# luisdiaz1997/GPzoo

Hardware: AMD Instinct MI355X
Metric: ELBO evals/sec (L=32-latent evaluations, all GPUs) at M=2048 inducing, N=200000, L=32 latents/GPU x 1 GPU(s) (higher is better)
Workload: dtype f32; 1 GPU; BASELINE configs[2]: Slide-seq-shaped synthetic, N=200000 spots, M=2048, L=32 latents/GPU x 1 GPU(s), matern32, f32; latents_total=32, whitened=True, chunk=0, factor_dtype=f64

## Files before the change

### gpzoo_amd/build.py

```python
from __future__ import annotations

import os
import subprocess
import sys

HERE = os.path.dirname(os.path.abspath(__file__))
CSRC = os.path.join(HERE, "csrc")
LIB = os.path.join(HERE, "libgpzoo_hip.so")
SOURCES = ["runtime.hip", "kfill.hip", "gemm.hip", "gemmw.hip", "gemmp.hip", "diag128.hip", "coop.hip", "factor.hip", "kgrad.hip", "mmops.hip", "poisson.hip", "svgp.hip", "vnngp.hip", "collective.hip", "spatial.hip", "nmf.hip", "smooth.hip", "kmeans.hip", "gram.hip", "poisson_sparse.hip", "nmf_sparse.hip", "deviance.hip", "nb.hip", "nb_sparse.hip", "nb_deviance.hip", "gaussian.hip", "gaussian_sparse.hip", "gene_rank.hip", "gene_dispersion.hip", "residual.hip", "moran_perm.hip", "spatial_stats.hip"]
HEADERS = ["common.h", "vec.h", "sparse_rows.h", "gene_rows.h", "moran_expr.h", "nb_passes.h", "moran_pass.h", "residual_gaussian.h", "gemm.h", "cov.h", "gemmw.h", "gemmp.h", "diag128.h", "factor.h", "kgrad.h", "mmops.h", os.path.join("..", "..", "include", "gpzoo_hip.h")]
FLAGS = ["--offload-arch=gfx950", "-O3", "-std=c++17", "-fPIC", "-ffp-contract=fast", "-Wall", "-Wno-unused-function"]
SOURCE_FLAGS = {"spatial.hip": ["-ffp-contract=off"], "smooth.hip": ["-ffp-contract=off"], "kmeans.hip": ["-ffp-contract=off"],
                "gene_rank.hip": ["-ffp-contract=off"], "gene_dispersion.hip": ["-ffp-contract=off"],
                "residual.hip": ["-ffp-contract=off"], "moran_perm.hip": ["-ffp-contract=off"],
                "spatial_stats.hip": ["-ffp-contract=off"]}


HASH_MARK = b"GPZ_SRC_HASH:"


def source_hash():
    import hashlib
    h = hashlib.sha256()
    for f in sorted(SOURCES + HEADERS):
        path = os.path.join(CSRC, f)
        if not os.path.exists(path):
            return None
        h.update(os.path.basename(f).encode() + b"\0")
        h.update(open(path, "rb").read())
        h.update(b"\0")
    return h.hexdigest()[:32]


def embedded_hash(lib_path: str = LIB):
    try:
        blob = open(lib_path, "rb").read()
    except OSError:
        return None
    i = blob.find(HASH_MARK)
    if i < 0:
        return None
    j = blob.find(b"\0", i)
    return blob[i + len(HASH_MARK):j].decode("ascii", "replace")
# ... 40 lines not shown
```

### gpzoo_amd/csrc/gemmw.h

```cpp
#pragma once
#include "common.h"

namespace gpz {

struct Fused1Args {
  const float* Linv; int64_t Mp;
  const float* Z; int64_t M;
  const float* X; int64_t nreal;
  int d, kind, L;
  const float* sigma; const float* ell;
  float* Wt; int64_t ncp;
  const float* muE;
  float* ps_sq; float* ps_mu;
};
bool fused1_supported(int dtype, int kind, int d);
int fused1_launch(const Fused1Args& a, hipStream_t s);

enum WideEpilogue {
  WIDE_STORE_STATS = 0,
  WIDE_STATS = 1,
  WIDE_STORE = 2,
  WIDE_STORE_COLSCALE = 3,
  WIDE_WBAR = 4,
  WIDE_KBAR = 5,
  WIDE_ADD_COLSCALE = 6,
};
struct WideArgs {
  const float* A; const float* B; int64_t Mp, ncp; int L;
  int upper, epilogue;
  float* C; const float* mu;
  float* ps_sq; float* ps_mu;
  const float* colscale; const float* colvec;
  const float* rowvec;
  const float* aux;
  const int32_t* gate;
};
bool wide_product_supported(int64_t Mp, int64_t ncp);
int wide_product_launch(const WideArgs& a, hipStream_t s);

bool wide_nt_supported(int64_t Mp, int64_t K);
int wide_nt_pieces(int64_t Mp, int64_t K, int L);
size_t wide_nt_scratch_floats(int64_t Mp, int64_t K, int L);
size_t wide_nt_vpart_floats(int64_t Mp, int64_t K, int L);
int wide_nt_launch(const float* A, const float* B, float* C, int64_t Mp, int64_t K, int L, hipStream_t s, float* scratch = nullptr,
                   const float* w = nullptr, const int32_t* gate = nullptr, const float* gm = nullptr, float* vpart = nullptr,
                   double* v = nullptr, int64_t v_stride = 0);

}
```

### gpzoo_amd/csrc/gemmw.hip

```cpp
#include "gemmw.h"

#include "cov.h"


#include <cmath>
#include <mutex>
#include <type_traits>
#include <utility>

#ifndef GPZ_W_ABL
#define GPZ_W_ABL 0
#endif

namespace gpz {

typedef float f32x4 __attribute__((ext_vector_type(4)));

enum { WB_MEM = 0, WB_GEN = 1 };
enum { WA_DENSE = 0, WA_LOWER = 1, WA_UPPER = 2 };
enum { WE_STORE_STATS = 0,
       WE_STATS = 1,
       WE_STORE = 2,
       WE_STORE_COLSCALE = 3,
       WE_WBAR = 4,
       WE_KBAR = 5,
       WE_ADD_COLSCALE = 6 };

struct WParams {
  const float* A; int64_t lda, sA0;
  const float* B; int64_t ldb, sB0;
  const float* Z; int64_t MD;
  const float* X; int64_t nreal;
  const float* sigma; const float* ell;
  float* C; int64_t ldc, sC0;
  const float* mu; int64_t sMu;
  float* ps_sq; float* ps_mu; int64_t ncols;
  const float* colscale; const float* colvec; int64_t sCs;
  const float* rowvec; int64_t sRv;
  const float* aux;
  int64_t M;
  int L, nblk, mtw, nt, W, strips;
  int pair, colmajor;
  const int32_t* gate;
};

constexpr int W_BK = 16;

template <int TM, int TN, int BSRC, int D>
struct WLds {
  static constexpr int A_ELEMS = TM * W_BK;
  static constexpr int RPP = 256 / TN;
  static constexpr int PITCH = 256 + (RPP == 2 ? 8 : RPP == 1 ? 4 : 16);
  static constexpr int B_ELEMS = (W_BK / RPP) * PITCH;
  static constexpr int STAGE = A_ELEMS + B_ELEMS;
  static constexpr int ZB = 128 * D;
  static constexpr size_t bytes = sizeof(float) * (2 * STAGE + (BSRC == WB_GEN ? 2 * ZB : 0));
};

template <int TM, int TN, int BSRC, int ATRI, int EPI, int KIND, int D>
// ... 222 lines not shown
    active = db < p.nblk && (int64_t)tj * TN + wn * 32 < p.ncols;
    n_a = 8 * (ATRI == WA_LOWER ? db : wm);
    fr_a = (wm * 128 + r) * BK + ((q ^ gperm(r)) * 4);
    step0 = k_begin / BK;
    t = 0;
    next_ti = leg + 1 < nlegs ? leg_ti[leg + 1] : -1;
#pragma unroll
    for (int mi = 0; mi < 8; ++mi)
#pragma unroll
      for (int ni = 0; ni < 2; ++ni) acc[mi][ni] = f32x4{0, 0, 0, 0};
    if constexpr (BSRC == WB_GEN) {
      z_load(step0 >> 3);
      asm volatile("s_waitcnt vmcnt(0)" ::: "memory");
      __syncthreads();
      b_generate(0, step0);
    }
    if (leg == 0) asm volatile("s_waitcnt vmcnt(0)" ::: "memory");
    asm volatile("s_waitcnt lgkmcnt(0)" ::: "memory");
    __builtin_amdgcn_s_barrier();
    if (!active) {
      idle_until(nk);
    } else if constexpr (ATRI == WA_DENSE) {
      full_until(nk);
    } else if constexpr (ATRI == WA_LOWER) {
      full_until(n_a);
      diagonal(diagonal, i0{});
      idle_until(nk);
    } else {
      idle_until(n_a);
      diagonal(diagonal, i0{});
      full_until(nk);
    }

    if (!active) continue;
    if (GPZ_W_ABL & 4) {
      float sum = 0.f;
#pragma unroll
      for (int mi = 0; mi < 8; ++mi)
#pragma unroll
        for (int ni = 0; ni < 2; ++ni)
#pragma unroll
          for (int g = 0; g < 4; ++g) sum += acc[mi][ni][g];
      if (sum == 12345.678f) p.ps_sq[0] = sum;
      continue;
    }
    const int64_t row0 = (int64_t)db * 128;
    const int64_t ccol0 = (int64_t)tj * TN + wn * 32;
    if (BSRC == WB_GEN && row0 + 128 > p.M) {
#pragma unroll
      for (int mi = 0; mi < 8; ++mi)
#pragma unroll
        for (int g = 0; g < 4; ++g)
          if (row0 + mi * 16 + 4 * q + g >= p.M) {
#pragma unroll
            for (int ni = 0; ni < 2; ++ni) acc[mi][ni][g] = 0.f;
          }
    }
    if constexpr (EPI == WE_STORE_STATS || EPI == WE_STATS) {
      float ssq[2] = {0.f, 0.f}, smu[2] = {0.f, 0.f};
#pragma unroll
      for (int mi = 0; mi < 8; ++mi) {
        f32x4 m4 = {0, 0, 0, 0};
        if constexpr (EPI == WE_STORE_STATS) m4 = *reinterpret_cast<const f32x4*>(p.mu + b0 * p.sMu + row0 + 4 * q + mi * 16);
#pragma unroll
        for (int g = 0; g < 4; ++g)
#pragma unroll
          for (int ni = 0; ni < 2; ++ni) {
            const float v = acc[mi][ni][g];
            ssq[ni] = __builtin_fmaf(v, v, ssq[ni]);
            if constexpr (EPI == WE_STORE_STATS) smu[ni] = __builtin_fmaf(m4[g], v, smu[ni]);
          }
      }
#pragma unroll
      for (int ni = 0; ni < 2; ++ni) {
        ssq[ni] += __shfl_xor(ssq[ni], 16); ssq[ni] += __shfl_xor(ssq[ni], 32);
        if constexpr (EPI == WE_STORE_STATS) { smu[ni] += __shfl_xor(smu[ni], 16); smu[ni] += __shfl_xor(smu[ni], 32); }
        if (q == 0) {
          const int64_t o = ((int64_t)b0 * p.nblk + db) * p.ncols + ccol0 + ni * 16 + r;
          p.ps_sq[o] = ssq[ni];
          if constexpr (EPI == WE_STORE_STATS) p.ps_mu[o] = smu[ni];
        }
      }
    }
    if constexpr (EPI != WE_STATS) {
      constexpr int LDE = 36;
      static_assert(NW * 16 * LDE <= G::STAGE, "the epilogue strips fit tile buffer 1");
      float* strip = sA(1) + wave * (16 * LDE);
      float* Cg = p.C + b0 * p.sC0 + row0 * p.ldc + ccol0;
      int srow = lane >> 3;
      asm volatile("" : "+v"(srow));
      const int c4 = (lane & 7) * 4;
      float cs[2] = {1.f, 1.f};
      if constexpr (EPI == WE_STORE_COLSCALE) {
#pragma unroll
        for (int ni = 0; ni < 2; ++ni) cs[ni] = p.colscale[b0 * p.sCs + ccol0 + ni * 16 + r];
      }
      f32x4 sc = {0, 0, 0, 0}, cv = {0, 0, 0, 0};
      if constexpr (EPI == WE_WBAR || EPI == WE_KBAR || EPI == WE_ADD_COLSCALE)
        sc = *reinterpret_cast<const f32x4*>(p.colscale + b0 * p.sCs + ccol0 + c4);
      if constexpr (EPI == WE_WBAR || EPI == WE_KBAR)
        cv = *reinterpret_cast<const f32x4*>(p.colvec + b0 * p.sCs + ccol0 + c4);
#pragma unroll
      for (int mi = 0; mi < 8; ++mi) {
#pragma unroll
        for (int ni = 0; ni < 2; ++ni)
#pragma unroll
          for (int g = 0; g < 4; ++g) strip[(4 * q + g) * LDE + ni * 16 + r] = cs[ni] * acc[mi][ni][g];
        __builtin_amdgcn_wave_barrier();
        f32x4 w[2];
        float rv[2];
        if constexpr (EPI == WE_WBAR || EPI == WE_KBAR || EPI == WE_ADD_COLSCALE) {
#pragma unroll
          for (int it = 0; it < 2; ++it) {
            const int64_t row = mi * 16 + it * 8 + srow;
            if constexpr (EPI == WE_WBAR) w[it] = *reinterpret_cast<const f32x4*>(p.aux + b0 * p.sC0 + (row0 + row) * p.ldc + ccol0 + c4);
            if constexpr (EPI == WE_ADD_COLSCALE) w[it] = *reinterpret_cast<const f32x4*>(Cg + (int64_t)row * p.ldc + c4);
            if constexpr (EPI != WE_ADD_COLSCALE) rv[it] = p.rowvec[b0 * p.sRv + row0 + row];
// ... 325 lines not shown
  GPZ_REQUIRE(fused1_supported(GPZ_F32, a.kind, a.d), "fused stage 1: kind=%d d=%d unsupported", a.kind, a.d);
  GPZ_REQUIRE(a.Mp % 128 == 0 && a.ncp % 128 == 0 && a.Mp > 0 && a.ncp > 0 && a.L > 0, "fused stage 1: bad extents");
  GPZ_REQUIRE(a.Mp * a.Mp * 4 < (1ll << 31) && a.M * a.d * 4 < (1ll << 31), "fused stage 1: M too large");
  constexpr int TM = 512, TN = 128;
  WParams p = {};
  p.A = a.Linv; p.lda = a.Mp; p.sA0 = a.Mp * a.Mp;
  p.Z = a.Z; p.MD = a.M * a.d; p.M = a.M;
  p.X = a.X; p.nreal = a.nreal;
  p.sigma = a.sigma; p.ell = a.ell;
  p.C = a.Wt; p.ldc = a.ncp; p.sC0 = a.Mp * a.ncp;
  p.mu = a.muE; p.sMu = a.Mp;
  p.ps_sq = a.ps_sq; p.ps_mu = a.ps_mu; p.ncols = a.ncp;
  p.L = a.L; p.nblk = (int)(a.Mp / 128); p.mtw = (int)((a.Mp + TM - 1) / TM); p.nt = (int)(a.ncp / TN);
  int strips = (p.nt + 31) / 32;
  const int want = (32 + p.mtw * p.L - 1) / (p.mtw * p.L);
  if (strips < want) strips = want < p.nt ? want : p.nt;
  p.W = (p.nt + strips - 1) / strips;
  p.strips = (p.nt + p.W - 1) / p.W;
  const int64_t units = (int64_t)p.mtw * p.L * p.strips;
  const int64_t nblocks = (units + 7) / 8 * 8 * p.W;
#define GPZ_W1(KIND, D) return launch_wide(gemmw_kernel<TM, TN, WB_GEN, WA_LOWER, WE_STORE_STATS, KIND, D>, \
                                           WLds<TM, TN, WB_GEN, D>::bytes, p, nblocks, s, 1024)
  if (a.kind == GPZ_KERNEL_MATERN32) { if (a.d == 2) GPZ_W1(1, 2); GPZ_W1(1, 1); }
  if (a.kind == GPZ_KERNEL_MATERN12) { if (a.d == 2) GPZ_W1(4, 2); GPZ_W1(4, 1); }
  if (a.kind == GPZ_KERNEL_MATERN52) { if (a.d == 2) GPZ_W1(5, 2); GPZ_W1(5, 1); }
  if (a.d == 2) GPZ_W1(0, 2);
  GPZ_W1(0, 1);
#undef GPZ_W1
}

bool wide_product_supported(int64_t Mp, int64_t ncp) {
  return Mp % 128 == 0 && ncp % 128 == 0 && Mp * Mp * 4 < (1ll << 31) && Mp * ncp * 4 < (1ll << 31);
}

template <int TM, int TN>
static int wide_product_launch_t(const WideArgs& a, hipStream_t s) {
  WParams p = {};
  p.A = a.A; p.lda = a.Mp; p.sA0 = a.Mp * a.Mp;
  p.B = a.B; p.ldb = a.ncp; p.sB0 = a.Mp * a.ncp;
  p.C = a.C; p.ldc = a.ncp; p.sC0 = a.Mp * a.ncp;
  p.mu = a.mu; p.sMu = a.Mp;
  p.ps_sq = a.ps_sq; p.ps_mu = a.ps_mu; p.ncols = a.ncp; p.M = a.Mp;
  p.colscale = a.colscale; p.colvec = a.colvec; p.sCs = a.ncp; p.rowvec = a.rowvec; p.sRv = a.Mp; p.aux = a.aux;
  p.gate = a.gate;
  p.L = a.L; p.nblk = (int)(a.Mp / 128); p.mtw = (int)((a.Mp + TM - 1) / TM); p.nt = (int)((a.ncp + TN - 1) / TN);
  constexpr int WMAX = 4096 / TN;
  int strips = (p.nt + WMAX - 1) / WMAX;
  const int want = (8 + p.L - 1) / p.L;
  if (strips < want) strips = want < p.nt ? want : p.nt;
  p.strips = strips;
  p.W = (p.nt + strips - 1) / strips;
  const int64_t units = (int64_t)p.L * p.strips;
  const int64_t paired = (units + 7) / 8 * 8 * ((p.mtw + 1) / 2) * p.W;
  p.pair = p.colmajor = paired >= 4 * 512;
  const int64_t nblocks = p.pair ? paired : (units + 7) / 8 * 8 * p.mtw * p.W;
  constexpr size_t lds = WLds<TM, TN, WB_MEM, 1>::bytes;
#define GPZ_WM(ATRI, EPI) return launch_wide(gemmw_kernel<TM, TN, WB_MEM, ATRI, EPI, 0, 1>, lds, p, nblocks, s)
  switch (a.epilogue) {
    case WIDE_STORE_STATS:
      GPZ_REQUIRE(!a.upper && a.C && a.mu && a.ps_sq && a.ps_mu, "wide product: store + statistics is the lower-triangular product and needs C, mu and both slabs");
      GPZ_WM(WA_LOWER, WE_STORE_STATS);
    case WIDE_STATS:
      GPZ_REQUIRE(a.upper && a.ps_sq, "wide product: statistics only is the upper-triangular product");
      GPZ_WM(WA_UPPER, WE_STATS);
    case WIDE_STORE:
      GPZ_REQUIRE(a.upper && a.C, "wide product: the plain store is built for the upper-triangular product");
      GPZ_WM(WA_UPPER, WE_STORE);
    case WIDE_STORE_COLSCALE:
      GPZ_REQUIRE(a.upper && a.C && a.colscale, "wide product: the column-scaled store is the upper-triangular product and needs the factors");
      GPZ_WM(WA_UPPER, WE_STORE_COLSCALE);
    case WIDE_WBAR:
      GPZ_REQUIRE(!a.upper && a.C && a.colscale && a.colvec && a.rowvec && a.aux, "wide product: the W-bar epilogue needs its operands");
      GPZ_WM(WA_LOWER, WE_WBAR);
    case WIDE_KBAR:
      GPZ_REQUIRE(a.upper == 2 && a.C && a.colscale && a.colvec && a.rowvec, "wide product: the K-bar epilogue is the dense product and needs its vectors");
      GPZ_WM(WA_DENSE, WE_KBAR);
    case WIDE_ADD_COLSCALE:
      GPZ_REQUIRE(a.upper == 1 && a.C && a.colscale, "wide product: the accumulating column-scaled store is the upper-triangular product");
      GPZ_WM(WA_UPPER, WE_ADD_COLSCALE);
    default: break;
  }
#undef GPZ_WM
  GPZ_REQUIRE(false, "wide product: unknown epilogue %d", a.epilogue);
}

int wide_product_launch(const WideArgs& a, hipStream_t s) {
  GPZ_REQUIRE(wide_product_supported(a.Mp, a.ncp) && a.L > 0, "wide product: bad extents");
  return wide_product_launch_t<128, 256>(a, s);
}

bool wide_nt_supported(int64_t Mp, int64_t K) {
  return Mp % 128 == 0 && K % 128 == 0 && K > 0 && Mp * K * 4 < (1ll << 31);
}

static bool nt_small_tiles(int64_t nblk) { return nblk <= 4; }
static int64_t nt_tiles(int64_t nblk) {
  if (nt_small_tiles(nblk)) return nblk * (nblk + 1) / 2;
  const int64_t mt = (nblk + 1) / 2;
  return mt * (mt + 1) - (nblk & 1);
}

int wide_nt_pieces(int64_t Mp, int64_t K, int L) {
  const int64_t tiles = nt_tiles(Mp / 128) * L;
  if (tiles >= 384) {
    const double r = (double)tiles / 512.0;
    int best = 1;
    double best_cost = 1e30;
    for (int S = 1; S <= 4; ++S) {
      if (S > 1 && K / S < 2048) break;
      const double rounds = r * S, cost = std::ceil(rounds - 1e-9) / rounds * (1.0 + 0.015 * (S - 1));
      if (cost < best_cost - 1e-9) { best_cost = cost; best = S; }
    }
// ... 56 lines not shown
```

### gpzoo_amd/csrc/kgrad.h

```cpp
#pragma once
#include "common.h"

namespace gpz {

struct KgradArgs {
  const void* Kbar; int64_t ld, stride;
  const void* Z; const void* X;
  const int64_t* gZ; const int64_t* gX;
  const void* sigma; const void* ell; const void* ga; const void* gr2;
  double gpow, scalar_scale;
  int64_t M, ncols, Mp;
  int d, G;
  double* acc;
};

int kgrad_launch(int dtype, int kind, const KgradArgs& a, int L, hipStream_t s);

}
```

### gpzoo_amd/csrc/kgrad.hip

```cpp
#include "kgrad.h"
#include "mmops.h"

namespace gpz {

__device__ __forceinline__ float kg_exp(float x) { return __builtin_amdgcn_exp2f(x * 1.44269504088896341f); }
__device__ __forceinline__ double kg_exp(double x) { return exp(x); }
__device__ __forceinline__ float kg_sqrt(float x) { return sqrtf(x); }
__device__ __forceinline__ double kg_sqrt(double x) { return sqrt(x); }
__device__ __forceinline__ float kg_rsqrt(float x) { return rsqrtf(x); }
__device__ __forceinline__ double kg_rsqrt(double x) { return 1.0 / sqrt(x); }
__device__ __forceinline__ float kg_pow(float x, float y) { return __builtin_amdgcn_exp2f(y * __builtin_amdgcn_logf(x)); }
__device__ __forceinline__ double kg_pow(double x, double y) { return pow(x, y); }

template <typename T, int KIND>
__global__ __launch_bounds__(256) void kgrad_kernel(KgradArgs a) {
  const int l = blockIdx.y, wave = threadIdx.x >> 6, lane = threadIdx.x & 63;
  const int64_t m = (int64_t)blockIdx.x * 4 + wave;
  if (m >= a.M) return;
  const T* kb = static_cast<const T*>(a.Kbar) + (int64_t)l * a.stride + m * a.ld;
  const T* Zp = static_cast<const T*>(a.Z);
  const T* Xp = static_cast<const T*>(a.X);
  const int d = a.d;
  const T sig = static_cast<const T*>(a.sigma)[l];
  const T ell = static_cast<const T*>(a.ell)[l];
  const T s2 = sig * sig, il2 = (T)1 / (ell * ell);
  T z[4] = {0, 0, 0, 0};
  for (int k = 0; k < d; ++k) z[k] = Zp[m * d + k];
  const int gz = (KIND == 2) ? ((uint64_t)a.gZ[m] < (uint64_t)a.G ? (int)a.gZ[m] : 0) : 0;
  const T aeff = (KIND == 2) ? static_cast<const T*>(a.ga)[l] : (T)0;
  const T gpow = (T)a.gpow;
  double dz[4] = {0, 0, 0, 0}, dsig = 0, dell = 0, da = 0;
  constexpr int UN = 4;
  for (int64_t c0 = lane; c0 < a.ncols; c0 += 64 * UN) {
    T g[UN], x[UN][4];
    int gx[UN];
#pragma unroll
    for (int u = 0; u < UN; ++u) {
      const int64_t c = c0 + 64 * u;
      const bool in = c < a.ncols;
      g[u] = in ? kb[c] : (T)0;
#pragma unroll
      for (int k = 0; k < 4; ++k) x[u][k] = (in && k < d) ? Xp[c * d + k] : (T)0;
      gx[u] = (KIND == 2 && in) ? ((uint64_t)a.gX[c] < (uint64_t)a.G ? (int)a.gX[c] : 0) : 0;
    }
    T pz[4] = {0, 0, 0, 0}, psig = 0, pell = 0, pa = 0;
#pragma unroll
    for (int u = 0; u < UN; ++u) {
      T diff[4], d2 = 0;
#pragma unroll
      for (int k = 0; k < 4; ++k) { diff[k] = (k < d) ? z[k] - x[u][k] : (T)0; d2 = fma(diff[k], diff[k], d2); }
      T cz;
      if (KIND == 0) {
        const T kv = s2 * kg_exp((T)-0.5 * d2 * il2);
        psig += g[u] * (T)2 * kv / sig;
        pell += g[u] * kv * d2 * il2 / ell;
        cz = -kv * il2;
      } else if (KIND == 1) {
        const T v = (T)1.7320508075688772935 * kg_sqrt(d2) / ell, e = kg_exp(-v);
        psig += g[u] * (T)2 * sig * ((T)1 + v) * e;
        pell += g[u] * s2 * v * v * e / ell;
        cz = -s2 * (T)3 * il2 * e;
      } else if (KIND == 4) {
        const T rr = kg_sqrt(d2), kv = s2 * kg_exp(-rr / ell);
        psig += g[u] * (T)2 * kv / sig;
        pell += g[u] * kv * rr * il2;
        cz = d2 > (T)0 ? -(kv / ell) * kg_rsqrt(d2) : (T)0;
      } else if (KIND == 5) {
        const T v = (T)2.2360679774997896964 * kg_sqrt(d2) / ell, e = kg_exp(-v), q3 = v * v / (T)3;
        psig += g[u] * (T)2 * sig * ((T)1 + v + q3) * e;
        pell += g[u] * s2 * q3 * ((T)1 + v) * e / ell;
        cz = -s2 * (T)5 / (T)3 * il2 * ((T)1 + v) * e;
      } else {
        const T r2 = static_cast<const T*>(a.gr2)[gz * a.G + gx[u]];
        const T den = aeff * r2 + (T)1;
        const T kv = s2 * kg_exp((T)-0.5 * d2 * il2 / den) * kg_pow(den, -gpow);
        psig += g[u] * (T)2 * kv / sig;
        pell += g[u] * kv * d2 * il2 / (ell * den);
        pa += g[u] * kv * ((T)0.5 * d2 * il2 / (den * den) - gpow / den) * r2;
        cz = -kv * il2 / den;
      }
      const T gc = g[u] * cz;
#pragma unroll
      for (int k = 0; k < 4; ++k) pz[k] = fma(gc, diff[k], pz[k]);
    }
    dsig += (double)psig; dell += (double)pell; da += (double)pa;
#pragma unroll
    for (int k = 0; k < 4; ++k) dz[k] += (double)pz[k];
  }
  double v[7] = {dz[0], dz[1], dz[2], dz[3], dsig * a.scalar_scale, dell * a.scalar_scale, da * a.scalar_scale};
#pragma unroll
  for (int i = 0; i < 7; ++i)
    for (int o = 32; o > 0; o >>= 1) v[i] += __shfl_down(v[i], o);
  if (lane == 0) {
    double* dst = a.acc + ((int64_t)l * a.Mp + m) * 8;
#pragma unroll
    for (int i = 0; i < 7; ++i) dst[i] += v[i];
  }
}

int kgrad_launch(int dtype, int kind, const KgradArgs& a, int L, hipStream_t s) {
  GPZ_REQUIRE((kind >= 0 && kind <= 2) || kind == GPZ_KERNEL_MATERN12 || kind == GPZ_KERNEL_MATERN52,
              "kgrad: unknown kernel kind %d", kind);
  dim3 grid((unsigned)((a.M + 3) / 4), (unsigned)L), block(256);
#define GPZ_KG(T, K) hipLaunchKernelGGL((kgrad_kernel<T, K>), grid, block, 0, s, a)
#define GPZ_KG_KINDS(T) \
  switch (kind) { case 0: GPZ_KG(T, 0); break; case 1: GPZ_KG(T, 1); break; case 4: GPZ_KG(T, 4); break; \
                  case 5: GPZ_KG(T, 5); break; default: GPZ_KG(T, 2); break; }
  if (dtype == GPZ_F32) GPZ_KG_KINDS(float) else GPZ_KG_KINDS(double)
#undef GPZ_KG_KINDS
#undef GPZ_KG
  GPZ_LAUNCH_OK();
  return 0;
}

}

extern "C" size_t gpz_kgrad_workspace_bytes(int64_t nA, int32_t n_latent) {
  if (nA < 1 || n_latent < 1) return 0;
  gpz::Carver c(nullptr);
  c.take<double>((int64_t)n_latent * nA * 8);
  return c.used();
}

extern "C" int gpz_kgrad(const gpz_kernel_desc* k, const void* A, int64_t nA, const void* B, int64_t nB, int32_t d,
                         const int64_t* gA, const int64_t* gB, const void* Kbar, int64_t ldk, int64_t stride_k,
                         double* grad_theta, double* grad_A, void* ws, size_t ws_bytes, void* stream) {
  using namespace gpz;
  GPZ_REQUIRE(k && A && B && Kbar && ws, "gpz_kgrad: null pointer");
  GPZ_REQUIRE(nA >= 1 && nB >= 1 && ldk >= nB && d >= 1 && d <= 4, "gpz_kgrad: bad extents nA=%lld nB=%lld ldk=%lld d=%d",
              (long long)nA, (long long)nB, (long long)ldk, d);
  GPZ_REQUIRE((k->kind >= 0 && k->kind <= 2) || k->kind == GPZ_KERNEL_MATERN12 || k->kind == GPZ_KERNEL_MATERN52,
              "gpz_kgrad: kernel kind %d has no parameters to differentiate", k->kind);
  GPZ_REQUIRE(k->n_latent >= 1 && (k->dtype == GPZ_F32 || k->dtype == GPZ_F64), "gpz_kgrad: bad kernel description");
  if (k->kind == GPZ_KERNEL_MGGP_RBF)
    GPZ_REQUIRE(gA && gB && k->group_a && k->group_r2 && k->n_groups >= 1, "gpz_kgrad: MGGP kernel needs groups, group_a, group_r2");
  GPZ_REQUIRE(ws_bytes >= gpz_kgrad_workspace_bytes(nA, k->n_latent), "gpz_kgrad: workspace too small");
  hipStream_t s = static_cast<hipStream_t>(stream);
  const int L = k->n_latent;
  Carver c(ws);
  double* acc = c.take<double>((int64_t)L * nA * 8);
  GPZ_HIP_OK(hipMemsetAsync(acc, 0, sizeof(double) * L * nA * 8, s));
  KgradArgs a;
  a.Kbar = Kbar; a.ld = ldk; a.stride = stride_k; a.Z = A; a.X = B; a.gZ = gA; a.gX = gB;
  a.sigma = k->sigma; a.ell = k->lengthscale; a.ga = k->group_a; a.gr2 = k->group_r2;
  a.gpow = k->group_pow; a.scalar_scale = 1.0; a.M = nA; a.ncols = nB; a.Mp = nA; a.d = d; a.G = k->n_groups; a.acc = acc;
  if (int rc = kgrad_launch(k->dtype, k->kind, a, L, s)) return rc;
  return kgrad_finish(acc, L, nA, nA, d, nullptr, grad_A, grad_theta, s);
// ... 2 lines not shown
```

### gpzoo_amd/csrc/svgp.hip

```cpp
#include "common.h"
#include "gemmw.h"
#include "gemmp.h"
#include "factor.h"
#include "gemm.h"
#include "kgrad.h"
#include "mmops.h"

#include <algorithm>
#include <cstdlib>
#include <cstring>

namespace gpz {

constexpr int NB = 128;

struct ProductSchedule { int cols, tpw; };
template <typename T>
static ProductSchedule product_schedule(bool stats_epilogue, int nt) {
  const int tpw = (sizeof(T) == 4 && stats_epilogue) ? 2 : 1;
  const int full = 16 * tpw;
  const int strips = (nt + full - 1) / full;
  int w = (nt + strips * tpw - 1) / (strips * tpw);
  if (w > 16) w = 16;
  return ProductSchedule{w * tpw, tpw};
// ... 845 lines not shown
    b.any_d = c.take<int32_t>(pl.nchunks + 1);
  }
  b.bytes = c.used();
  return b;
}

template <typename TR, typename T>
__global__ __launch_bounds__(256) void q_finish_kernel(TR* __restrict__ R, const T* __restrict__ Hd, int64_t Mp, int64_t M,
                                                      const double* __restrict__ u, const double* __restrict__ v) {
  const int l = blockIdx.z;
  const int64_t i = blockIdx.y, j = (int64_t)blockIdx.x * 256 + threadIdx.x;
  if (j >= Mp || (j >> 7) > (i >> 7)) return;
  const int64_t o = (int64_t)l * Mp * Mp + i * Mp + j;
  double r = (double)R[o];
  if (Hd) r += (double)Hd[o];
  if (i < M && j < M) r += u[(int64_t)l * Mp + i] * v[(int64_t)l * Mp + j];
  R[o] = (TR)r;
}
template <typename T>
__global__ void minus_identity_t_kernel(T* __restrict__ A, int64_t Mp) {
  const int l = blockIdx.y;
  const int64_t i = (int64_t)blockIdx.x * 256 + threadIdx.x;
  if (i < Mp) A[(int64_t)l * Mp * Mp + i * (Mp + 1)] -= (T)1;
}

static bool backward_algebra(int64_t N, int64_t Mp, bool full, int flags, bool f64_algebra) {
  static const int env = [] { const char* e = getenv("GPZ_SVGP_BACKWARD"); return !e ? 0 : !strcmp(e, "algebra") ? 1 : !strcmp(e, "classic") ? 2 : 0; }();
  if (flags & GPZ_SVGP_BACKWARD_ALGEBRA) return true;
  if (flags & GPZ_SVGP_BACKWARD_CLASSIC) return false;
  if (env) return env == 1;
  return full ? 10 * N >= (f64_algebra ? 44 : 22) * Mp : 4 * N >= 3 * Mp;
}

template <typename T>
static int svgp_backward_t(const gpz_svgp_problem* p, const gpz_svgp_grads* g, int64_t chunk, void* ws, size_t ws_bytes,
                           hipStream_t s) {
  const Plan pl = make_plan(p, chunk);
  const bool wh = p->whitened != 0;
  const bool full = g->grad_theta != nullptr || g->grad_Z != nullptr;
  Buffers<T> b = carve<T>(pl, wh, ws);
  BwdBuffers<T> w = carve_bwd<T>(pl, wh, full, ws, b.bytes);
  GPZ_REQUIRE(ws_bytes >= w.bytes, "gpz_svgp_backward: workspace too small (%zu < %zu)", ws_bytes, w.bytes);
  const int64_t L = pl.L, M = pl.M, Mp = pl.Mp, N = pl.N, mm = Mp * Mp;
  const int L32 = (int)L;
  const bool alg64 = sizeof(T) == 4 && !wh;
  const bool alg = backward_algebra(N, Mp, full, p->flags, alg64);
  gpz_svgp_problem q = *p;
  q.chol = nullptr; q.Lu = nullptr;
  if (int rc = prepare_t<T>(&q, pl, b, s)) return rc;
  {
    Zeroer z;
    if (alg) z.add(w.H, sizeof(T) * L * mm);
    z.add(w.G, sizeof(T) * L * mm);
    if (!wh) z.add(w.G2, sizeof(T) * L * mm);
    if (full) {
      if (alg && wh) {
        z.add(w.Hd, sizeof(T) * L * mm);
        z.add(w.any_d, sizeof(int32_t) * (pl.nchunks + 1));
      }
      if (!alg) z.add(w.GL, sizeof(T) * L * mm);
      z.add(w.kacc, sizeof(double) * L * Mp * 8);
      z.add(w.sig_direct, sizeof(double) * L);
    }
    if (int rc = z.run(s)) return rc;
  }
  const dim3 g32((unsigned)(Mp / 32), (unsigned)(Mp / 32), L32);
// ... 124 lines not shown
      if (with_hd)
        if (int rc = syrk(w.csd, w.Hd, w.any_d + ci)) return rc;
      v_done = wide_nt;
    } else {
      bool done = false;
      if constexpr (sizeof(T) == 4) {
        if (wide) {
          WideArgs wa = {};
          wa.A = b.LuT; wa.B = Wc; wa.Mp = Mp; wa.ncp = ncp; wa.L = L32; wa.upper = 1; wa.epilogue = WIDE_STORE_COLSCALE;
          wa.C = w.Pc; wa.colscale = w.cs;
          if (int rc = wide_product_launch(wa, s)) return rc;
          done = true;
        }
      }
      if (!done) {
        GemmParams<T> g2;
        g2.A = b.LuT; g2.lda = Mp; g2.sA0 = mm;
        g2.B = Wc; g2.ldb = ncp; g2.sB0 = Mp * ncp;
        g2.C = w.Pc; g2.ldc = ncp; g2.sC0 = Mp * ncp;
        g2.nb0 = L32; g2.mt = (int)pl.nblk; g2.nt = nt; g2.K = (int)Mp; g2.flags = GF_A_UPPER | GF_GROUP_COLS;
        g2.super_cols = sched_plain.cols; g2.colscale = w.cs; g2.sCs = ncp; g2.ncols = ncp;
        if (int rc = gemm_launch(g2, EPI_STORE_COLSCALE, s)) return rc;
      }
      if (wide_nt) {
        if constexpr (sizeof(T) == 4) { if (int rc = wide_nt_launch(Wc, w.Pc, w.G, Mp, ncp, L32, s, w.nt_part)) return rc; }
      } else if (int rc = nt_generic(Wc, w.Pc, w.G)) return rc;
    }
    if (!v_done) {
      hipLaunchKernelGGL((rowdot_kernel<T>), dim3((unsigned)(Mp / 4), L32), dim3(256), 0, s, Wc, Mp, ncp,
                         static_cast<const T*>(g->g_mean), N, n0, w.mu_part, pl.nchunks, ci);
      GPZ_LAUNCH_OK();
    }
    if (full) {
      bool done = false;
      if constexpr (sizeof(T) == 4) {
        if (wide && alg) {
          WideArgs wk = {};
          wk.A = w.A1; wk.B = Wc; wk.Mp = Mp; wk.ncp = ncp; wk.L = L32; wk.upper = 2; wk.epilogue = WIDE_KBAR;
          wk.C = w.Pc; wk.colscale = w.cs; wk.colvec = w.gmc; wk.rowvec = w.a3;
          if (int rc = wide_product_launch(wk, s)) return rc;
          if (with_hd) {
            WideArgs wc = {};
            wc.A = w.LinvT; wc.B = Wc; wc.Mp = Mp; wc.ncp = ncp; wc.L = L32; wc.upper = 1; wc.epilogue = WIDE_ADD_COLSCALE;
            wc.C = w.Pc; wc.colscale = w.csd; wc.gate = w.any_d + ci;
            if (int rc = wide_product_launch(wc, s)) return rc;
          }
          done = true;
        }
        if (wide && !alg) {
          WideArgs wa = {};
          wa.A = w.LuN; wa.B = w.Pc; wa.Mp = Mp; wa.ncp = ncp; wa.L = L32; wa.upper = 0; wa.epilogue = WIDE_WBAR;
          wa.C = b.Kc; wa.colscale = w.csc; wa.colvec = w.gmc; wa.rowvec = b.muE; wa.aux = Wc;
          if (int rc = wide_product_launch(wa, s)) return rc;
          WideArgs wb = {};
          wb.A = w.LinvT; wb.B = b.Kc; wb.Mp = Mp; wb.ncp = ncp; wb.L = L32; wb.upper = 1; wb.epilogue = WIDE_STORE;
          wb.C = w.Pc;
          if (int rc = wide_product_launch(wb, s)) return rc;
          done = true;
        }
      }
      if (!done) {
        if (alg) {
          GemmParams<T> g2;
          g2.A = b.LuT; g2.lda = Mp; g2.sA0 = mm;
          g2.B = Wc; g2.ldb = ncp; g2.sB0 = Mp * ncp;
          g2.C = w.Pc; g2.ldc = ncp; g2.sC0 = Mp * ncp;
          g2.nb0 = L32; g2.mt = (int)pl.nblk; g2.nt = nt; g2.K = (int)Mp; g2.flags = GF_A_UPPER | GF_GROUP_COLS;
          g2.super_cols = sched_plain.cols; g2.colscale = w.cs; g2.sCs = ncp; g2.ncols = ncp;
          if (int rc = gemm_launch(g2, EPI_STORE_COLSCALE, s)) return rc;
        }
        GemmParams<T> g4;
        g4.A = w.LuN; g4.lda = Mp; g4.sA0 = mm;
        g4.B = w.Pc; g4.ldb = ncp; g4.sB0 = Mp * ncp;
        g4.C = b.Kc; g4.ldc = ncp; g4.sC0 = Mp * ncp;
        g4.nb0 = L32; g4.mt = (int)pl.nblk; g4.nt = nt; g4.K = (int)Mp; g4.flags = GF_A_LOWER | GF_GROUP_COLS;
        g4.super_cols = sched_plain.cols; g4.colscale = w.csc; g4.colvec = w.gmc; g4.sCs = ncp; g4.rowvec = b.muE; g4.sRv = Mp;
        g4.aux = Wc; g4.ncols = ncp;
        if (int rc = gemm_launch(g4, EPI_WBAR, s)) return rc;
        GemmParams<T> g5;
        g5.A = w.LinvT; g5.lda = Mp; g5.sA0 = mm;
        g5.B = b.Kc; g5.ldb = ncp; g5.sB0 = Mp * ncp;
        g5.C = w.Pc; g5.ldc = ncp; g5.sC0 = Mp * ncp;
        g5.nb0 = L32; g5.mt = (int)pl.nblk; g5.nt = nt; g5.K = (int)Mp; g5.flags = GF_A_UPPER | GF_GROUP_COLS;
        g5.super_cols = sched_plain.cols;
        if (int rc = gemm_launch(g5, EPI_STORE, s)) return rc;
      }
      if (!alg) {
        if (wide_nt) {
          if constexpr (sizeof(T) == 4) { if (int rc = wide_nt_launch(w.Pc, Wc, w.GL, Mp, ncp, L32, s, w.nt_part)) return rc; }
        } else if (int rc = nt_generic(w.Pc, Wc, w.GL)) return rc;
      }
      KgradArgs ka;
      ka.Kbar = w.Pc; ka.ld = ncp; ka.stride = Mp * ncp; ka.Z = p->Z; ka.X = Xc;
      ka.gZ = p->gZ; ka.gX = p->gX ? p->gX + n0 : nullptr;
      ka.sigma = p->k.sigma; ka.ell = p->k.lengthscale; ka.ga = p->k.group_a; ka.gr2 = p->k.group_r2;
      ka.gpow = p->k.group_pow; ka.scalar_scale = 1.0; ka.M = M; ka.ncols = nreal; ka.Mp = Mp; ka.d = p->d;
      ka.G = p->k.n_groups; ka.acc = w.kacc;
      if (int rc = kgrad_launch(p->dtype, p->k.kind, ka, L32, s)) return rc;
      hipLaunchKernelGGL((sigma_direct_kernel<T>), dim3(L32), dim3(256), 0, s, w.csc, ncp,
                         static_cast<const T*>(p->k.sigma), w.sig_direct);
      GPZ_LAUNCH_OK();
    }
  }
  hipLaunchKernelGGL(chunk_sum_kernel, dim3((unsigned)((Mp + 255) / 256), L32), dim3(256), 0, s, w.mu_part, pl.nchunks,
                     Mp, w.mu_sum);
  GPZ_LAUNCH_OK();
  if (alg) {
    hipLaunchKernelGGL((mirror_lower_kernel<T>), g32, dim3(256), 0, s, w.H, Mp);
    GPZ_LAUNCH_OK();
    if (int rc = tgemm(w.H, b.LuT, w.G, GF_B_TRANS | GF_B_LOWER | GF_TILES_LOWER)) return rc;
    if (full) {
      if (alg64) {
        hipLaunchKernelGGL((widen_kernel<T>), dim3(2048), dim3(256), 0, s, (const T*)w.H, w.D1, L * mm, 0);
        GPZ_LAUNCH_OK();
        if (int rc = dgemm(w.D2, w.D1, w.D3, GF_TILES_LOWER)) return rc;
        hipLaunchKernelGGL((q_finish_kernel<double, T>), gm, dim3(256), 0, s, w.D3, (const T*)nullptr, Mp, M,
                           (const double*)w.me, (const double*)w.mu_sum);
        GPZ_LAUNCH_OK();
        if (int rc = tril_transpose(b.Linv, Mp, L32, w.D1, s)) return rc;
        if (int rc = dgemm(w.D1, w.D3, w.D4, GF_A_UPPER | GF_TILES_LOWER)) return rc;
      } else {
        if (int rc = tgemm(w.SwI, w.H, w.PS, GF_TILES_LOWER)) return rc;
        hipLaunchKernelGGL((q_finish_kernel<T, T>), gm, dim3(256), 0, s, w.PS, wh ? (const T*)w.Hd : (const T*)nullptr, Mp, M,
                           (const double*)w.me, (const double*)w.mu_sum);
        GPZ_LAUNCH_OK();
        if (int rc = tgemm(w.LinvT, w.PS, w.GL, GF_A_UPPER | GF_TILES_LOWER)) return rc;
      }
    }
  }
  const double* g_kl = g->g_kl;
  if (g_kl && !wh) {
// ... 263 lines not shown
```

Baseline: 2.650 ELBO evals/s.

## Fuse kernel-gradient contraction into wide K-bar product epilogue

Result: no change. 2.645 ELBO evals/s (-0.2%).

```diff
diff --git a/gpzoo_amd/build.py b/gpzoo_amd/build.py
--- a/gpzoo_amd/build.py
+++ b/gpzoo_amd/build.py
@@ -8,7 +8,7 @@
 CSRC = os.path.join(HERE, "csrc")
 LIB = os.path.join(HERE, "libgpzoo_hip.so")
 SOURCES = ["runtime.hip", "kfill.hip", "gemm.hip", "gemmw.hip", "gemmp.hip", "diag128.hip", "coop.hip", "factor.hip", "kgrad.hip", "mmops.hip", "poisson.hip", "svgp.hip", "vnngp.hip", "collective.hip", "spatial.hip", "nmf.hip", "smooth.hip", "kmeans.hip", "gram.hip", "poisson_sparse.hip", "nmf_sparse.hip", "deviance.hip", "nb.hip", "nb_sparse.hip", "nb_deviance.hip", "gaussian.hip", "gaussian_sparse.hip", "gene_rank.hip", "gene_dispersion.hip", "residual.hip", "moran_perm.hip", "spatial_stats.hip"]
-HEADERS = ["common.h", "vec.h", "sparse_rows.h", "gene_rows.h", "moran_expr.h", "nb_passes.h", "moran_pass.h", "residual_gaussian.h", "gemm.h", "cov.h", "gemmw.h", "gemmp.h", "diag128.h", "factor.h", "kgrad.h", "mmops.h", os.path.join("..", "..", "include", "gpzoo_hip.h")]
+HEADERS = ["common.h", "vec.h", "sparse_rows.h", "gene_rows.h", "moran_expr.h", "nb_passes.h", "moran_pass.h", "residual_gaussian.h", "gemm.h", "cov.h", "gemmw.h", "gemmp.h", "diag128.h", "factor.h", "kgrad.h", "kgrad_terms.h", "mmops.h", os.path.join("..", "..", "include", "gpzoo_hip.h")]
 FLAGS = ["--offload-arch=gfx950", "-O3", "-std=c++17", "-fPIC", "-ffp-contract=fast", "-Wall", "-Wno-unused-function"]
 SOURCE_FLAGS = {"spatial.hip": ["-ffp-contract=off"], "smooth.hip": ["-ffp-contract=off"], "kmeans.hip": ["-ffp-contract=off"],
                 "gene_rank.hip": ["-ffp-contract=off"], "gene_dispersion.hip": ["-ffp-contract=off"],
diff --git a/gpzoo_amd/csrc/gemmw.h b/gpzoo_amd/csrc/gemmw.h
--- a/gpzoo_amd/csrc/gemmw.h
+++ b/gpzoo_amd/csrc/gemmw.h
@@ -24,6 +24,8 @@
   WIDE_WBAR = 4,
   WIDE_KBAR = 5,
   WIDE_ADD_COLSCALE = 6,
+  WIDE_KBAR_CONTRACT = 7,
+  WIDE_COLSCALE_CONTRACT = 8,
 };
 struct WideArgs {
   const float* A; const float* B; int64_t Mp, ncp; int L;
@@ -34,8 +36,12 @@
   const float* rowvec;
   const float* aux;
   const int32_t* gate;
+  const float* Z; const float* X; const float* sigma; const float* ell;
+  int64_t M, nreal; int d, kind;
 };
 bool wide_product_supported(int64_t Mp, int64_t ncp);
+bool wide_contract_supported(int kind, int d);
+size_t wide_contract_part_floats(int64_t Mp, int64_t ncp, int L);
 int wide_product_launch(const WideArgs& a, hipStream_t s);
 
 bool wide_nt_supported(int64_t Mp, int64_t K);
diff --git a/gpzoo_amd/csrc/gemmw.hip b/gpzoo_amd/csrc/gemmw.hip
--- a/gpzoo_amd/csrc/gemmw.hip
+++ b/gpzoo_amd/csrc/gemmw.hip
@@ -1,7 +1,7 @@
 #include "gemmw.h"
 
 #include "cov.h"
-
+#include "kgrad_terms.h"
 
 #include <cmath>
 #include <mutex>
@@ -24,7 +24,9 @@
        WE_STORE_COLSCALE = 3,
        WE_WBAR = 4,
        WE_KBAR = 5,
-       WE_ADD_COLSCALE = 6 };
+       WE_ADD_COLSCALE = 6,
+       WE_KBAR_CONTRACT = 7,
+       WE_COLSCALE_CONTRACT = 8 };
 
 struct WParams {
   const float* A; int64_t lda, sA0;
@@ -313,7 +315,8 @@
       full_until(nk);
     }
 
-    if (!active) continue;
+    constexpr bool CONTRACT = EPI == WE_KBAR_CONTRACT || EPI == WE_COLSCALE_CONTRACT;
+    if (!active && !CONTRACT) continue;
     if (GPZ_W_ABL & 4) {
       float sum = 0.f;
 #pragma unroll
@@ -363,7 +366,78 @@
         }
       }
     }
-    if constexpr (EPI != WE_STATS) {
+    if constexpr (CONTRACT) {
+      static_assert(!CONTRACT || (BSRC == WB_MEM && WMW == 1 && NW * 512 <= G::STAGE), "one 128-row block per workgroup; the sums fit tile buffer 1");
+      static_assert(!CONTRACT || D == 1 || D == 2, "dz0, dz1");
+      float* const red = sA(1);
+      const KgHoist kh = kg_hoist<KIND>(p.sigma[b0], p.ell[b0]);
+      if (active) {
+        float xn[2][D], csn[2], cvn[2];
+        bool creal[2];
+#pragma unroll
+        for (int ni = 0; ni < 2; ++ni) {
+          const int64_t n = ccol0 + ni * 16 + r;
+          creal[ni] = n < p.nreal;
+#pragma unroll
+          for (int k = 0; k < D; ++k) xn[ni][k] = creal[ni] ? p.X[n * D + k] : 0.f;
+          csn[ni] = creal[ni] ? p.colscale[b0 * p.sCs + n] : 0.f;
+          cvn[ni] = (EPI == WE_KBAR_CONTRACT && creal[ni]) ? p.colvec[b0 * p.sCs + n] : 0.f;
+        }
+#pragma unroll
+        for (int mi = 0; mi < 8; ++mi) {
+          int rbase = (int)row0 + mi * 16 + 4 * q;
+          asm volatile("" : "+v"(rbase));
+          float a[16];
+#pragma unroll
+          for (int g = 0; g < 4; ++g) {
+            const int row = rbase + g;
+            const bool rreal = row < p.M;
+            const float* zp = p.Z + (rreal ? row : 0) * D;
+            float z[D];
+#pragma unroll
+            for (int k = 0; k < D; ++k) z[k] = zp[k];
+            const float rv = EPI == WE_KBAR_CONTRACT ? p.rowvec[b0 * p.sRv + row] : 0.f;
+            float sz[2] = {0.f, 0.f}, ssig = 0.f, sell = 0.f;
+#pragma unroll
+            for (int ni = 0; ni < 2; ++ni) {
+              float v = acc[mi][ni][g] * csn[ni];
+              if constexpr (EPI == WE_KBAR_CONTRACT) v += rv * cvn[ni];
+              v = (creal[ni] && rreal) ? v : 0.f;
+              float diff[D], d2 = 0.f;
+#pragma unroll
+              for (int k = 0; k < D; ++k) { diff[k] = z[k] - xn[ni][k]; d2 = __builtin_fmaf(diff[k], diff[k], d2); }
+              float e, wz, wsig, well;
+              kg_weights<KIND>(kh, d2, e, wz, wsig, well);
+              const float t = v * e, tz = t * wz;
+#pragma unroll
+              for (int k = 0; k < D; ++k) sz[k] = __builtin_fmaf(tz, diff[k], sz[k]);
+              ssig = __builtin_fmaf(t, wsig, ssig);
+              sell = __builtin_fmaf(t, well, sell);
+            }
+            a[g * 4 + 0] = sz[0]; a[g * 4 + 1] = sz[1]; a[g * 4 + 2] = ssig; a[g * 4 + 3] = sell;
+          }
+#pragma unroll
+          for (int i = 0; i < 8; ++i) { const bool up = r & 8; const float send = up ? a[i] : a[i + 8]; a[i] = (up ? a[i + 8] : a[i]) + __shfl_xor(send, 8); }
+#pragma unroll
+          for (int i = 0; i < 4; ++i) { const bool up = r & 4; const float send = up ? a[i] : a[i + 4]; a[i] = (up ? a[i + 4] : a[i]) + __shfl_xor(send, 4); }
+#pragma unroll
+          for (int i = 0; i < 2; ++i) { const bool up = r & 2; const float send = up ? a[i] : a[i + 2]; a[i] = (up ? a[i + 2] : a[i]) + __shfl_xor(send, 2); }
+          { const bool up = r & 1; const float send = up ? a[0] : a[1]; a[0] = (up ? a[1] : a[0]) + __shfl_xor(send, 1); }
+          red[(wave * 8 + mi) * 64 + lane] = a[0];
+        }
+      } else {
+#pragma unroll
+        for (int mi = 0; mi < 8; ++mi) red[(wave * 8 + mi) * 64 + lane] = 0.f;
+      }
+      asm volatile("s_waitcnt lgkmcnt(0)" ::: "memory");
+      __builtin_amdgcn_s_barrier();
+      float tot = 0.f;
+#pragma unroll
+      for (int w = 0; w < NW; ++w) tot += red[w * 512 + tid];
+      const int qty = tid & 3;
+      p.C[(((int64_t)b0 * p.nt + tj) * Mp + row0) * 4 + tid] = tot * (qty < 2 ? kh.sz : qty == 2 ? kh.ssig : kh.sell);
+    }
+    if constexpr (EPI != WE_STATS && !CONTRACT) {
       constexpr int LDE = 36;
       static_assert(NW * 16 * LDE <= G::STAGE, "the epilogue strips fit tile buffer 1");
       float* strip = sA(1) + wave * (16 * LDE);
@@ -755,6 +829,10 @@
 bool wide_product_supported(int64_t Mp, int64_t ncp) {
   return Mp % 128 == 0 && ncp % 128 == 0 && Mp * Mp * 4 < (1ll << 31) && Mp * ncp * 4 < (1ll << 31);
 }
+
+bool wide_contract_supported(int kind, int d) { return fused1_supported(GPZ_F32, kind, d); }
+
+size_t wide_contract_part_floats(int64_t Mp, int64_t ncp, int L) { return (size_t)L * (size_t)((ncp + 255) / 256) * (size_t)Mp * 4; }
 
 template <int TM, int TN>
 static int wide_product_launch_t(const WideArgs& a, hipStream_t s) {
@@ -801,6 +879,23 @@
     case WIDE_ADD_COLSCALE:
       GPZ_REQUIRE(a.upper == 1 && a.C && a.colscale, "wide product: the accumulating column-scaled store is the upper-triangular product");
       GPZ_WM(WA_UPPER, WE_ADD_COLSCALE);
+    case WIDE_KBAR_CONTRACT:
+    case WIDE_COLSCALE_CONTRACT: {
+      const bool kbar = a.epilogue == WIDE_KBAR_CONTRACT;
+      GPZ_REQUIRE(a.upper == (kbar ? 2 : 1) && a.C && a.colscale && (!kbar || (a.colvec && a.rowvec)),
+                  "wide product: the contracting epilogue is the dense K-bar product or its upper-triangular correction and needs their vectors");
+      GPZ_REQUIRE(wide_contract_supported(a.kind, a.d) && a.Z && a.X && a.sigma && a.ell && a.M >= 1 && a.M <= a.Mp &&
+                  a.nreal >= 1 && a.nreal <= a.ncp, "wide product: the contracting epilogue needs a stationary kernel on 1-D / 2-D inputs");
+      p.Z = a.Z; p.MD = a.M * a.d; p.M = a.M; p.X = a.X; p.nreal = a.nreal; p.sigma = a.sigma; p.ell = a.ell;
+#define GPZ_WC(KIND, D) do { if (kbar) return launch_wide(gemmw_kernel<TM, TN, WB_MEM, WA_DENSE, WE_KBAR_CONTRACT, KIND, D>, lds, p, nblocks, s); \
+                             return launch_wide(gemmw_kernel<TM, TN, WB_MEM, WA_UPPER, WE_COLSCALE_CONTRACT, KIND, D>, lds, p, nblocks, s); } while (0)
+      if (a.kind == GPZ_KERNEL_MATERN32) { if (a.d == 2) GPZ_WC(1, 2); GPZ_WC(1, 1); }
+      if (a.kind == GPZ_KERNEL_MATERN12) { if (a.d == 2) GPZ_WC(4, 2); GPZ_WC(4, 1); }
+      if (a.kind == GPZ_KERNEL_MATERN52) { if (a.d == 2) GPZ_WC(5, 2); GPZ_WC(5, 1); }
+      if (a.d == 2) GPZ_WC(0, 2);
+      GPZ_WC(0, 1);
+#undef GPZ_WC
+    }
     default: break;
   }
 #undef GPZ_WM
diff --git a/gpzoo_amd/csrc/kgrad.h b/gpzoo_amd/csrc/kgrad.h
--- a/gpzoo_amd/csrc/kgrad.h
+++ b/gpzoo_amd/csrc/kgrad.h
@@ -16,4 +16,7 @@
 
 int kgrad_launch(int dtype, int kind, const KgradArgs& a, int L, hipStream_t s);
 
+int kpart_reduce_launch(const float* part, const float* part2, const int32_t* gate, int nt, int64_t Mp, int64_t M, int L,
+                        double* acc, hipStream_t s);
+
 }
diff --git a/gpzoo_amd/csrc/kgrad.hip b/gpzoo_amd/csrc/kgrad.hip
--- a/gpzoo_amd/csrc/kgrad.hip
+++ b/gpzoo_amd/csrc/kgrad.hip
@@ -1,16 +1,8 @@
 #include "kgrad.h"
+#include "kgrad_terms.h"
 #include "mmops.h"
 
 namespace gpz {
-
-__device__ __forceinline__ float kg_exp(float x) { return __builtin_amdgcn_exp2f(x * 1.44269504088896341f); }
-__device__ __forceinline__ double kg_exp(double x) { return exp(x); }
-__device__ __forceinline__ float kg_sqrt(float x) { return sqrtf(x); }
-__device__ __forceinline__ double kg_sqrt(double x) { return sqrt(x); }
-__device__ __forceinline__ float kg_rsqrt(float x) { return rsqrtf(x); }
-__device__ __forceinline__ double kg_rsqrt(double x) { return 1.0 / sqrt(x); }
-__device__ __forceinline__ float kg_pow(float x, float y) { return __builtin_amdgcn_exp2f(y * __builtin_amdgcn_logf(x)); }
-__device__ __forceinline__ double kg_pow(double x, double y) { return pow(x, y); }
 
 template <typename T, int KIND>
 __global__ __launch_bounds__(256) void kgrad_kernel(KgradArgs a) {
@@ -50,26 +42,8 @@
 #pragma unroll
       for (int k = 0; k < 4; ++k) { diff[k] = (k < d) ? z[k] - x[u][k] : (T)0; d2 = fma(diff[k], diff[k], d2); }
       T cz;
-      if (KIND == 0) {
-        const T kv = s2 * kg_exp((T)-0.5 * d2 * il2);
-        psig += g[u] * (T)2 * kv / sig;
-        pell += g[u] * kv * d2 * il2 / ell;
-        cz = -kv * il2;
-      } else if (KIND == 1) {
-        const T v = (T)1.7320508075688772935 * kg_sqrt(d2) / ell, e = kg_exp(-v);
-        psig += g[u] * (T)2 * sig * ((T)1 + v) * e;
-        pell += g[u] * s2 * v * v * e / ell;
-        cz = -s2 * (T)3 * il2 * e;
-      } else if (KIND == 4) {
-        const T rr = kg_sqrt(d2), kv = s2 * kg_exp(-rr / ell);
-        psig += g[u] * (T)2 * kv / sig;
-        pell += g[u] * kv * rr * il2;
-        cz = d2 > (T)0 ? -(kv / ell) * kg_rsqrt(d2) : (T)0;
-      } else if (KIND == 5) {
-        const T v = (T)2.2360679774997896964 * kg_sqrt(d2) / ell, e = kg_exp(-v), q3 = v * v / (T)3;
-        psig += g[u] * (T)2 * sig * ((T)1 + v + q3) * e;
-        pell += g[u] * s2 * q3 * ((T)1 + v) * e / ell;
-        cz = -s2 * (T)5 / (T)3 * il2 * ((T)1 + v) * e;
+      if constexpr (KIND != 2) {
+        cz = kg_terms<T, KIND>(g[u], d2, sig, ell, s2, il2, psig, pell);
       } else {
         const T r2 = static_cast<const T*>(a.gr2)[gz * a.G + gx[u]];
         const T den = aeff * r2 + (T)1;
@@ -113,6 +87,32 @@
   return 0;
 }
 
+__global__ __launch_bounds__(256) void kpart_reduce_kernel(const float* __restrict__ part, const float* __restrict__ part2,
+                                                           const int32_t* __restrict__ gate, int nt, int64_t Mp, int64_t M,
+                                                           double* __restrict__ acc) {
+  const int l = blockIdx.y;
+  const int64_t i = (int64_t)blockIdx.x * 256 + threadIdx.x, m = i >> 2;
+  const int qty = (int)(i & 3);
+  if (m >= M) return;
+  double t = 0.0;
+  const float* src = part + ((int64_t)l * nt * Mp + m) * 4 + qty;
+  for (int tile = 0; tile < nt; ++tile) t += (double)src[(int64_t)tile * Mp * 4];
+  if (part2 && *gate != 0) {
+    src = part2 + ((int64_t)l * nt * Mp + m) * 4 + qty;
+    for (int tile = 0; tile < nt; ++tile) t += (double)src[(int64_t)tile * Mp * 4];
+  }
+  acc[((int64_t)l * Mp + m) * 8 + (qty < 2 ? qty : qty + 2)] += t;
+}
+
+int kpart_reduce_launch(const float* part, const float* part2, const int32_t* gate, int nt, int64_t Mp, int64_t M, int L,
+                        double* acc, hipStream_t s) {
+  GPZ_REQUIRE(part && acc && nt >= 1 && M >= 1 && M <= Mp && L >= 1 && (!part2 || gate), "kernel-gradient partials: bad arguments");
+  hipLaunchKernelGGL(kpart_reduce_kernel, dim3((unsigned)((M * 4 + 255) / 256), (unsigned)L), dim3(256), 0, s, part, part2,
+                     gate, nt, Mp, M, acc);
+  GPZ_LAUNCH_OK();
+  return 0;
+}
+
 }
 
 extern "C" size_t gpz_kgrad_workspace_bytes(int64_t nA, int32_t n_latent) {
diff --git a/gpzoo_amd/csrc/kgrad_terms.h b/gpzoo_amd/csrc/kgrad_terms.h
--- /dev/null
+++ b/gpzoo_amd/csrc/kgrad_terms.h
@@ -0,0 +1,90 @@
+#pragma once
+#include <hip/hip_runtime.h>
+
+namespace gpz {
+
+__device__ __forceinline__ float kg_exp(float x) { return __builtin_amdgcn_exp2f(x * 1.44269504088896341f); }
+__device__ __forceinline__ double kg_exp(double x) { return exp(x); }
+__device__ __forceinline__ float kg_sqrt(float x) { return sqrtf(x); }
+__device__ __forceinline__ double kg_sqrt(double x) { return sqrt(x); }
+__device__ __forceinline__ float kg_rsqrt(float x) { return rsqrtf(x); }
+__device__ __forceinline__ double kg_rsqrt(double x) { return 1.0 / sqrt(x); }
+__device__ __forceinline__ float kg_pow(float x, float y) { return __builtin_amdgcn_exp2f(y * __builtin_amdgcn_logf(x)); }
+__device__ __forceinline__ double kg_pow(double x, double y) { return pow(x, y); }
+
+template <typename T, int KIND>
+__device__ __forceinline__ T kg_terms(T g, T d2, T sig, T ell, T s2, T il2, T& psig, T& pell) {
+  static_assert(KIND == 0 || KIND == 1 || KIND == 4 || KIND == 5, "stationary kinds only");
+  T cz;
+  if (KIND == 0) {
+    const T kv = s2 * kg_exp((T)-0.5 * d2 * il2);
+    psig += g * (T)2 * kv / sig;
+    pell += g * kv * d2 * il2 / ell;
+    cz = -kv * il2;
+  } else if (KIND == 1) {
+    const T v = (T)1.7320508075688772935 * kg_sqrt(d2) / ell, e = kg_exp(-v);
+    psig += g * (T)2 * sig * ((T)1 + v) * e;
+    pell += g * s2 * v * v * e / ell;
+    cz = -s2 * (T)3 * il2 * e;
+  } else if (KIND == 4) {
+    const T rr = kg_sqrt(d2), kv = s2 * kg_exp(-rr / ell);
+    psig += g * (T)2 * kv / sig;
+    pell += g * kv * rr * il2;
+    cz = d2 > (T)0 ? -(kv / ell) * kg_rsqrt(d2) : (T)0;
+  } else {
+    const T v = (T)2.2360679774997896964 * kg_sqrt(d2) / ell, e = kg_exp(-v), q3 = v * v / (T)3;
+    psig += g * (T)2 * sig * ((T)1 + v + q3) * e;
+    pell += g * s2 * q3 * ((T)1 + v) * e / ell;
+    cz = -s2 * (T)5 / (T)3 * il2 * ((T)1 + v) * e;
+  }
+  return cz;
+}
+
+struct KgHoist {
+  float cv, ce;
+  float sz, ssig, sell;
+};
+
+template <int KIND>
+__device__ __forceinline__ KgHoist kg_hoist(float sig, float ell) {
+  static_assert(KIND == 0 || KIND == 1 || KIND == 4 || KIND == 5, "stationary kinds only");
+  constexpr float LOG2E = 1.44269504088896341f;
+  const float il = 1.f / ell, s2 = sig * sig, il2 = il * il;
+  KgHoist h;
+  h.ssig = 2.f * sig;
+  if (KIND == 0) {
+    h.cv = 0.f; h.ce = -0.5f * il2 * LOG2E;
+    h.sz = -s2 * il2; h.sell = s2 * il2 * il;
+  } else if (KIND == 4) {
+    h.cv = 0.f; h.ce = il * LOG2E;
+    h.sz = -s2 * il; h.sell = s2 * il2;
+  } else {
+    h.cv = (KIND == 1 ? 1.7320508075688772935f : 2.2360679774997896964f) * il; h.ce = h.cv * LOG2E;
+    h.sz = (KIND == 1 ? -3.f : -5.f / 3.f) * s2 * il2; h.sell = s2 * il;
+  }
+  return h;
+}
+
+template <int KIND>
+__device__ __forceinline__ void kg_weights(const KgHoist& h, float d2, float& e, float& wz, float& wsig, float& well) {
+  if (KIND == 0) {
+    e = __builtin_amdgcn_exp2f(h.ce * d2);
+    wz = 1.f; wsig = 1.f; well = d2;
+  } else if (KIND == 4) {
+    const float rr = __builtin_amdgcn_sqrtf(d2);
+    e = __builtin_amdgcn_exp2f(-(h.ce * rr));
+    wz = d2 >= 1.17549435e-38f ? __builtin_amdgcn_rsqf(d2) : 0.f;
+    wsig = 1.f; well = rr;
+  } else {
+    const float rr = __builtin_amdgcn_sqrtf(d2), v = h.cv * rr;
+    e = __builtin_amdgcn_exp2f(-(h.ce * rr));
+    if (KIND == 1) {
+      wz = 1.f; wsig = 1.f + v; well = v * v;
+    } else {
+      const float q3 = v * v * 0.333333333333333333f;
+      wz = 1.f + v; wsig = wz + q3; well = q3 * wz;
+    }
+  }
+}
+
+}
diff --git a/gpzoo_amd/csrc/svgp.hip b/gpzoo_amd/csrc/svgp.hip
--- a/gpzoo_amd/csrc/svgp.hip
+++ b/gpzoo_amd/csrc/svgp.hip
@@ -901,6 +901,13 @@
   return full ? 10 * N >= (f64_algebra ? 44 : 22) * Mp : 4 * N >= 3 * Mp;
 }
 
+static bool kbar_contract(const gpz_svgp_problem* p) {
+  if (p->gZ || p->gX || !wide_contract_supported(p->k.kind, p->d)) return false;
+  const char* e = getenv("GPZ_SVGP_KBAR");
+  if (e && !strcmp(e, "store")) return false;
+  return true;
+}
+
 template <typename T>
 static int svgp_backward_t(const gpz_svgp_problem* p, const gpz_svgp_grads* g, int64_t chunk, void* ws, size_t ws_bytes,
                            hipStream_t s) {
@@ -1091,9 +1098,31 @@
       GPZ_LAUNCH_OK();
     }
     if (full) {
-      bool done = false;
+      bool done = false, contracted = false;
       if constexpr (sizeof(T) == 4) {
-        if (wide && alg) {
+        if (wide && alg && kbar_contract(p)) {
+          const size_t pf = wide_contract_part_floats(Mp, ncp, L32);
+          GPZ_REQUIRE(2 * pf <= (size_t)(L * Mp * pl.nc), "gpz_svgp_backward: the kernel-gradient partials do not fit the Pbar buffer");
+          float* part = reinterpret_cast<float*>(w.Pc);
+          WideArgs wk = {};
+          wk.A = w.A1; wk.B = Wc; wk.Mp = Mp; wk.ncp = ncp; wk.L = L32; wk.upper = 2; wk.epilogue = WIDE_KBAR_CONTRACT;
+          wk.C = part; wk.colscale = w.cs; wk.colvec = w.gmc; wk.rowvec = w.a3;
+          wk.Z = static_cast<const float*>(p->Z); wk.X = static_cast<const float*>(Xc);
+          wk.sigma = static_cast<const float*>(p->k.sigma); wk.ell = static_cast<const float*>(p->k.lengthscale);
+          wk.M = M; wk.nreal = nreal; wk.d = p->d; wk.kind = p->k.kind;
+          if (int rc = wide_product_launch(wk, s)) return rc;
+          if (with_hd) {
+            WideArgs wc = wk;
+            wc.A = w.LinvT; wc.upper = 1; wc.epilogue = WIDE_COLSCALE_CONTRACT;
+            wc.C = part + pf; wc.colscale = w.csd; wc.colvec = nullptr; wc.rowvec = nullptr; wc.gate = w.any_d + ci;
+            if (int rc = wide_product_launch(wc, s)) return rc;
+          }
+          if (int rc = kpart_reduce_launch(part, with_hd ? part + pf : nullptr, with_hd ? w.any_d + ci : nullptr,
+                                           (int)((ncp + 255) / 256), Mp, M, L32, w.kacc, s))
+            return rc;
+          done = contracted = true;
+        }
+        if (wide && alg && !done) {
           WideArgs wk = {};
           wk.A = w.A1; wk.B = Wc; wk.Mp = Mp; wk.ncp = ncp; wk.L = L32; wk.upper = 2; wk.epilogue = WIDE_KBAR;
           wk.C = w.Pc; wk.colscale = w.cs; wk.colvec = w.gmc; wk.rowvec = w.a3;
@@ -1149,13 +1178,15 @@
           if constexpr (sizeof(T) == 4) { if (int rc = wide_nt_launch(w.Pc, Wc, w.GL, Mp, ncp, L32, s, w.nt_part)) return rc; }
         } else if (int rc = nt_generic(w.Pc, Wc, w.GL)) return rc;
       }
-      KgradArgs ka;
-      ka.Kbar = w.Pc; ka.ld = ncp; ka.stride = Mp * ncp; ka.Z = p->Z; ka.X = Xc;
-      ka.gZ = p->gZ; ka.gX = p->gX ? p->gX + n0 : nullptr;
-      ka.sigma = p->k.sigma; ka.ell = p->k.lengthscale; ka.ga = p->k.group_a; ka.gr2 = p->k.group_r2;
-      ka.gpow = p->k.group_pow; ka.scalar_scale = 1.0; ka.M = M; ka.ncols = nreal; ka.Mp = Mp; ka.d = p->d;
-      ka.G = p->k.n_groups; ka.acc = w.kacc;
-      if (int rc = kgrad_launch(p->dtype, p->k.kind, ka, L32, s)) return rc;
+      if (!contracted) {
+        KgradArgs ka;
+        ka.Kbar = w.Pc; ka.ld = ncp; ka.stride = Mp * ncp; ka.Z = p->Z; ka.X = Xc;
+        ka.gZ = p->gZ; ka.gX = p->gX ? p->gX + n0 : nullptr;
+        ka.sigma = p->k.sigma; ka.ell = p->k.lengthscale; ka.ga = p->k.group_a; ka.gr2 = p->k.group_r2;
+        ka.gpow = p->k.group_pow; ka.scalar_scale = 1.0; ka.M = M; ka.ncols = nreal; ka.Mp = Mp; ka.d = p->d;
+        ka.G = p->k.n_groups; ka.acc = w.kacc;
+        if (int rc = kgrad_launch(p->dtype, p->k.kind, ka, L32, s)) return rc;
+      }
       hipLaunchKernelGGL((sigma_direct_kernel<T>), dim3(L32), dim3(256), 0, s, w.csc, ncp,
                          static_cast<const T*>(p->k.sigma), w.sig_direct);
       GPZ_LAUNCH_OK();
```
